# glacierbliss/iceberg_tracking_code

Hardware: AMD Instinct MI355X
Metric: frame_pairs_per_sec (higher is better)
Workload: dtype u8/int32/f32

## Files before the change

iceberg_tracking_code_amd/csrc/k_corners.hip:

```cpp
#include <algorithm>
#include <climits>
#include <cstdlib>

#include "icelk_internal.h"
#include "strip_sqrt.h"

namespace icelk {

namespace {

__device__ __forceinline__ int reflect101(int p, int n)
{
    if (n == 1) return 0;
    while (p < 0 || p >= n) p = p < 0 ? -p : 2 * n - 2 - p;
    return p;
}

__device__ __forceinline__ unsigned ordered_key(float v)
{
    const unsigned b = __float_as_uint(v);
    return (b & 0x80000000u) ? ~b : (b | 0x80000000u);
}
__device__ __forceinline__ float key_to_float(unsigned k)
{
    const unsigned b = (k & 0x80000000u) ? (k & 0x7fffffffu) : ~k;
    return __uint_as_float(b);
}

__device__ __forceinline__ unsigned pack_xy(int x, int y) { return ((unsigned)y << 16) | (unsigned)x; }

__device__ __forceinline__ float threshold_of(const unsigned* max_key, double quality)
{
    const unsigned mk = *max_key;
    const double max_val = mk ? (double)key_to_float(mk) : 0.0;
    return (float)(max_val * quality);
}

__device__ __forceinline__ float row_smooth(float a, float b, float c, float k0, float k1, int variant)
{
    if (variant & 2) return fmaf(k1, c, fmaf(k0, b, __fmul_rn(k1, a)));
    return __fadd_rn(__fadd_rn(__fmul_rn(k1, a), __fmul_rn(k0, b)), __fmul_rn(k1, c));
}

__device__ __forceinline__ void sobel_cov(float a0, float b0, float c0, float a1, float c1, float a2, float b2,
                                          float c2, float k0, float k1, float& xx, float& xy, float& yy, int variant = 0)
{
    const float dx = (variant & 1) ? fmaf(__fadd_rn(__fsub_rn(c0, a0), __fsub_rn(c2, a2)), k1, __fmul_rn(__fsub_rn(c1, a1), k0))
                                   : __fadd_rn(__fmul_rn(__fadd_rn(__fsub_rn(c0, a0), __fsub_rn(c2, a2)), k1),
                                               __fmul_rn(__fsub_rn(c1, a1), k0));
    const float t0 = row_smooth(a0, b0, c0, k0, k1, variant);
    const float t2 = row_smooth(a2, b2, c2, k0, k1, variant);
    const float dy = __fsub_rn(t2, t0);
    xx = __fmul_rn(dx, dx);
    xy = __fmul_rn(dx, dy);
    yy = __fmul_rn(dy, dy);
}

typedef float f2 __attribute__((ext_vector_type(2)));
__device__ __forceinline__ void sobel_cov2(f2 a0, f2 b0, f2 c0, f2 a1, f2 c1, f2 a2, f2 b2, f2 c2, float k0, float k1,
                                           f2& xx, f2& xy, f2& yy)
{
    const f2 dx = ((c0 - a0) + (c2 - a2)) * k1 + (c1 - a1) * k0;
    const f2 t0 = (a0 * k1 + b0 * k0) + c0 * k1;
    const f2 t2 = (a2 * k1 + b2 * k0) + c2 * k1;
    const f2 dy = t2 - t0;
    xx = dx * dx;
    xy = dx * dy;
    yy = dy * dy;
}

template <int N, int BS>
__device__ __forceinline__ void window_sums(const double (&v)[N + BS - 1], double (&out)[N])
{
    if constexpr (BS <= 3) {
#pragma unroll
        for (int i = 0; i < N; i++) {
            double s = 0;
#pragma unroll
            for (int k = 0; k < BS; k++) s += v[i + k];
            out[i] = s;
        }
    } else {
        double s = v[0];
#pragma unroll
        for (int k = 1; k < BS; k++) s += v[k];
        out[0] = s;
#pragma unroll
        for (int i = 1; i < N; i++) {
            s = (s - v[i - 1]) + v[i + BS - 1];
            out[i] = s;
        }
    }
}

__device__ __forceinline__ float min_eig_of(double s0, double s1, double s2, int variant = 0)
{
    const float a = __fmul_rn((float)s0, 0.5f), b = (float)s1, c = __fmul_rn((float)s2, 0.5f);
    const float d = __fsub_rn(a, c);
    const float r = (variant & 4) ? fmaf(b, b, __fmul_rn(d, d)) : __fadd_rn(__fmul_rn(d, d), __fmul_rn(b, b));
    return __fsub_rn(__fadd_rn(a, c), sqrtf(r));
}

__device__ __forceinline__ void publish_max(unsigned* max_key, unsigned best, int tid)
{
#pragma unroll
    for (int o = 32; o >= 1; o >>= 1) {
        const unsigned other = __shfl_xor(best, o);
        best = other > best ? other : best;
    }
    if ((tid & 63) == 0 && best > __atomic_load_n(max_key, __ATOMIC_RELAXED)) atomicMax(max_key, best);
}

struct CandSrc {
    const unsigned long long* keys;
    const int* blk_count;
    int nblk;
    int region;
};

constexpr int gcd_c(int a, int b) { return b == 0 ? a : gcd_c(b, a % b); }

template <int BS>
struct StripCfg {
    static constexpr int NT = 256;
    static constexpr int AN = BS / 2;
    static constexpr int EW = NT - (BS - 1);
    static constexpr int TW = EW - 2;
    static constexpr int R = 4;
    static constexpr int UNROLL = BS * R / gcd_c(BS, R);
    static constexpr int EH = (64 / UNROLL) * UNROLL;
    static constexpr int SH = EH - 2;
    static constexpr int NROWS = EH + BS - 1;
    static constexpr int RX = 4;
    static constexpr int NG = (EW + RX - 1) / RX;
    static constexpr int VP = NT + 2;
    static constexpr int SUB = 16, NSUB = (SH + SUB - 1) / SUB;
    static constexpr int V_BYTES = R * 3 * VP * 8;
    static constexpr int E_BYTES = 8 * NT * 4;
    static constexpr int LDS_BYTES = V_BYTES + E_BYTES;
    static_assert(EH % R == 0 && NG <= 64 && RX * NG <= NT + RX - 1, "one wave per row of a batch");
    static_assert(RX * (NG - 1) + RX + BS - 2 < VP, "row tasks stay inside a row of column sums");
    static_assert((VP * 8) % 16 == 0, "16-byte reads of the column sums");
};

struct PixelRow {
    __amdgpu_buffer_rsrc_t rsrc;
    unsigned at;
    __device__ __forceinline__ unsigned operator[](unsigned x) const { return __builtin_amdgcn_raw_buffer_load_b8(rsrc, x, at, 0); }
};
struct PixelRows {
    __amdgpu_buffer_rsrc_t rsrc;
    unsigned pitch;
    __device__ __forceinline__ PixelRow row(int y) const { return PixelRow{rsrc, (unsigned)y * pitch}; }
};

struct SobelRoll {
    float d1, d2, t1, t2;
};

__device__ __forceinline__ float smooth3(float a, float b, float c, float k0, float k1)
{
    return __fadd_rn(__fadd_rn(__fmul_rn(k1, a), __fmul_rn(k0, b)), __fmul_rn(k1, c));
}

template <int N, bool BAND>
__device__ __forceinline__ void min_eig_strip(const double (&Sm)[3][N], float (&e)[N])
{
    if constexpr (!BAND) {
#pragma unroll
        for (int k = 0; k < N; k++) e[k] = min_eig_of(Sm[0][k], Sm[1][k], Sm[2][k]);
        return;
    }
    float tr[N], r[N];
    unsigned lo = 0xffffffffu, hi = 0u;
#pragma unroll
    for (int k = 0; k < N; k++) {
        const float a = __fmul_rn((float)Sm[0][k], 0.5f), b = (float)Sm[1][k], c = __fmul_rn((float)Sm[2][k], 0.5f);
        const float d = __fsub_rn(a, c);
        r[k] = __fadd_rn(__fmul_rn(d, d), __fmul_rn(b, b));
        tr[k] = __fadd_rn(a, c);
        const unsigned rb = __float_as_uint(r[k]);
        lo = rb < lo ? rb : lo;
        hi = rb > hi ? rb : hi;
    }
    if (__builtin_expect(__builtin_amdgcn_ballot_w64(lo < SQRT_BAND_LO || hi > SQRT_BAND_HI) == 0, 1)) {
#pragma unroll
        for (int k = 0; k < N; k++) e[k] = __fsub_rn(tr[k], sqrt_in_band(r[k]));
    } else {
#pragma unroll
        for (int k = 0; k < N; k++) e[k] = __fsub_rn(tr[k], sqrtf(r[k]));
    }
}

template <int BS, bool FRESH, bool FAST>
__device__ __forceinline__ void strip_body(const uint8_t* __restrict__ img, int w, int h, int pitch, float k0, float k1,
                                           const uint8_t* __restrict__ mask, int mask_pitch, unsigned* __restrict__ max_key,
                                           unsigned long long* __restrict__ raw, int* __restrict__ blk_count,
                                           float* __restrict__ eig_out, uint8_t* smem, int* s_cnt)
{
    using C = StripCfg<BS>;
    double* Vb = reinterpret_cast<double*>(smem);
    float* Er = reinterpret_cast<float*>(smem + C::V_BYTES);
    const int tid = threadIdx.x;
    const int x0 = blockIdx.x * C::TW, y0 = blockIdx.y * C::SH;
    const int xs = x0 - 1 - C::AN, ys = y0 - 1 - C::AN;
    const int rx = reflect101(xs + tid, w);
    const unsigned xm = (unsigned)reflect101(rx - 1, w), xc = (unsigned)rx, xp = (unsigned)reflect101(rx + 1, w);
    const PixelRows px{__builtin_amdgcn_make_buffer_rsrc(const_cast<uint8_t*>(img), 0, pitch * h, 0x00020000), (unsigned)pitch};
    const int bid = blockIdx.y * gridDim.x + blockIdx.x;
    if (tid < C::NSUB) s_cnt[tid] = 0;
    if (tid < C::R * 3 * (C::VP - C::NT)) Vb[(tid / (C::VP - C::NT)) * C::VP + C::NT + tid % (C::VP - C::NT)] = 0.0;

    float ring[3][BS];
#pragma unroll
    for (int k = 0; k < BS; k++) ring[0][k] = ring[1][k] = ring[2][k] = 0.f;
    double V[3] = {0.0, 0.0, 0.0};
    SobelRoll S{};
    unsigned pa = 0, pb = 0, pc = 0;
    if (!FRESH) {
        const PixelRow r2 = px.row(ys - 1), r1 = px.row(ys), r0 = px.row(ys + 1);
        const float a2 = (float)r2[xm], b2 = (float)r2[xc], c2 = (float)r2[xp];
        const float a1 = (float)r1[xm], b1 = (float)r1[xc], c1 = (float)r1[xp];
        S.d2 = __fsub_rn(c2, a2); S.t2 = smooth3(a2, b2, c2, k0, k1);
        S.d1 = __fsub_rn(c1, a1); S.t1 = smooth3(a1, b1, c1, k0, k1);
        pa = r0[xm]; pb = r0[xc]; pc = r0[xp];
    }
    auto cov_row = [&](int r, float& xx, float& xy, float& yy) {
        float dtop, dmid, dbot, ttop, tbot;
        if (FRESH) {
            const int ry = reflect101(ys + r, h);
            const PixelRow q0 = px.row(reflect101(ry - 1, h)), q1 = px.row(ry), q2 = px.row(reflect101(ry + 1, h));
            const float a0 = (float)q0[xm], b0 = (float)q0[xc], c0 = (float)q0[xp];
            const float a1 = (float)q1[xm], c1 = (float)q1[xp];
            const float a2 = (float)q2[xm], b2 = (float)q2[xc], c2 = (float)q2[xp];
            dtop = __fsub_rn(c0, a0); dmid = __fsub_rn(c1, a1); dbot = __fsub_rn(c2, a2);
            ttop = smooth3(a0, b0, c0, k0, k1); tbot = smooth3(a2, b2, c2, k0, k1);
        } else {
            float a = (float)pa, b = (float)pb, c = (float)pc;
            asm("" : "+v"(a), "+v"(c));
            int nr = ys + r + 2;
            nr = nr < h ? nr : h - 1;
            const PixelRow q = px.row(nr);
            pa = q[xm]; pb = q[xc]; pc = q[xp];
            dtop = S.d2; dmid = S.d1; dbot = __fsub_rn(c, a);
            ttop = S.t2; tbot = smooth3(a, b, c, k0, k1);
            S.d2 = S.d1; S.d1 = dbot; S.t2 = S.t1; S.t1 = tbot;
        }
        const float dx = __fadd_rn(__fmul_rn(__fadd_rn(dtop, dbot), k1), __fmul_rn(dmid, k0));
        const float dy = __fsub_rn(tbot, ttop);
        xx = __fmul_rn(dx, dx); xy = __fmul_rn(dx, dy); yy = __fmul_rn(dy, dy);
    };

#pragma unroll
    for (int r = 0; r < BS - 1; r++) {
        float p[3];
        cov_row(r, p[0], p[1], p[2]);
#pragma unroll
        for (int q = 0; q < 3; q++) { V[q] += (double)p[q]; ring[q][r] = p[q]; }
    }

    unsigned best = 0;
    constexpr int KL = C::TW - C::RX * (C::NG - 1);
    static_assert(KL >= 0 && KL < C::RX && C::RX * C::NG - 1 >= C::TW, "the last row task holds the strip's last output column");
    int top_hi[3], top_lo[3];
#pragma unroll
    for (int k = 0; k < 3; k++) { top_hi[k] = INT_MIN; top_lo[k] = INT_MAX; }
    const int wr = __builtin_amdgcn_readfirstlane(tid >> 6), g = tid & 63;
    for (int base = 0; base < C::EH; base += C::UNROLL) {
#pragma unroll
        for (int j = 0; j < C::UNROLL; j++) {
            const int i = base + j;
            const int K = (BS - 1 + j) % BS;
            float p[3];
            cov_row(BS - 1 + i, p[0], p[1], p[2]);
#pragma unroll
            for (int q = 0; q < 3; q++) {
                V[q] = (V[q] + (double)p[q]) - (double)ring[q][K];
                ring[q][K] = p[q];
                Vb[((j % C::R) * 3 + q) * C::VP + tid] = V[q];
            }
            __builtin_amdgcn_sched_barrier(0);
            if (j % C::R != C::R - 1) continue;
            const int eb = i / C::R;
            __syncthreads();
            if (g < C::NG && wr < C::R) {
                double Sm[3][C::RX];
#pragma unroll
                for (int q = 0; q < 3; q++) {
                    double v[C::RX + BS - 1];
                    const double* src = Vb + (wr * 3 + q) * C::VP + C::RX * g;
#pragma unroll
                    for (int k = 0; k < C::RX + BS - 1; k++) v[k] = src[k];
                    window_sums<C::RX, BS>(v, Sm[q]);
                    __builtin_amdgcn_sched_barrier(0);
                }
                const int er = eb * C::R + wr;
                float e[C::RX];
                min_eig_strip<C::RX, BS != 3>(Sm, e);
                *reinterpret_cast<float4*>(Er + (er & 7) * C::NT + C::RX * g) = make_float4(e[0], e[1], e[2], e[3]);
                const int y = y0 - 1 + er;
                if constexpr (FAST) {
                    if (er >= 1 && er <= C::SH) {
#pragma unroll
                        for (int k = 0; k < C::RX; k++) {
                            const int cls = k == 0 ? 0 : (k <= KL ? 1 : 2), bits = __float_as_int(e[k]);
                            top_hi[cls] = max(top_hi[cls], bits);
                            top_lo[cls] = min(top_lo[cls], bits);
                        }
                    }
                } else if (er >= 1 && er <= C::SH && y < h) {
#pragma unroll
                    for (int k = 0; k < C::RX; k++) {
                        const int ce = C::RX * g + k, x = x0 - 1 + ce;
                        if (ce >= 1 && ce <= C::TW && x < w) {
                            if (eig_out) eig_out[(size_t)y * w + x] = e[k];
                            if (!mask || mask[(size_t)y * mask_pitch + x]) {
                                const unsigned key = ordered_key(e[k]);
                                best = key > best ? key : best;
                            }
                        }
                    }
                }
            }
            __syncthreads();
            {
                const int x = x0 - 1 + tid;
                if (tid >= 1 && tid <= C::TW && x >= 1 && x < w - 1) {
                    float m3[6], mid[6], side[6];
#pragma unroll
                    for (int k = 0; k < 6; k++) {
                        const float* row = Er + ((eb * C::R - 2 + k) & 7) * C::NT + tid;
                        const float l = row[-1], c = row[0], r = row[1];
                        mid[k] = c;
                        side[k] = fmaxf(l, r);
                        m3[k] = fmaxf(side[k], c);
                    }
#pragma unroll
                    for (int q = 0; q < 4; q++) {
                        const int c = eb * C::R - 1 + q, y = y0 - 1 + c;
                        if (c < 1 || c > C::SH || y < 1 || y >= h - 1) continue;
                        const float v = mid[q + 1];
                        if (!(v > 0.f)) continue;
                        const float m = fmaxf(fmaxf(m3[q], m3[q + 2]), side[q + 1]);
                        if (v < m) continue;
                        if (mask && !mask[(size_t)y * mask_pitch + x]) continue;
                        const int sub = (c - 1) / C::SUB;
                        const int pos = atomicAdd(&s_cnt[sub], 1);
                        raw[((size_t)bid * C::NSUB + sub) * (C::TW * C::SUB) + pos] =
                            ((unsigned long long)ordered_key(v) << 32) | pack_xy(x, y);
                    }
                }
            }
        }
    }
    if constexpr (FAST) {
        const bool counts[3] = {g >= 1 && g < C::NG, g < C::NG, g < C::NG - 1};
        int hi = INT_MIN, lo = INT_MAX;
#pragma unroll
        for (int k = 0; k < 3; k++)
            if (counts[k]) { hi = max(hi, top_hi[k]); lo = min(lo, top_lo[k]); }
        if (lo <= hi) best = ordered_key(__int_as_float(hi >= 0 ? hi : lo));
    }
    publish_max(max_key, best, tid);
    __syncthreads();
    if (tid < C::NSUB) blk_count[bid * C::NSUB + tid] = s_cnt[tid];
}

template <int BS>
__global__ __launch_bounds__(256) __attribute__((amdgpu_waves_per_eu(3, 4))) void k_eig_strip(const uint8_t* __restrict__ img, int w, int h, int pitch, float k0,
                                                    float k1, const uint8_t* __restrict__ mask, int mask_pitch,
                                                    unsigned* __restrict__ max_key,
                                                    unsigned long long* __restrict__ raw, int* __restrict__ blk_count,
                                                    float* __restrict__ eig_out)
{
    using C = StripCfg<BS>;
    extern __shared__ __attribute__((aligned(16))) uint8_t smem[];
    __shared__ int s_cnt[C::NSUB];
    const int ys = (int)blockIdx.y * C::SH - 1 - C::AN;
    const bool rolling = ys - 1 >= 0 && ys + C::NROWS <= h - 1;
    const bool inside_x = ((int)blockIdx.x + 1) * C::TW <= w;
    if (rolling && inside_x && !mask && !eig_out)
        strip_body<BS, false, true>(img, w, h, pitch, k0, k1, mask, mask_pitch, max_key, raw, blk_count, eig_out, smem, s_cnt);
    else if (rolling)
        strip_body<BS, false, false>(img, w, h, pitch, k0, k1, mask, mask_pitch, max_key, raw, blk_count, eig_out, smem, s_cnt);
    else
        strip_body<BS, true, false>(img, w, h, pitch, k0, k1, mask, mask_pitch, max_key, raw, blk_count, eig_out, smem, s_cnt);
}

__device__ __forceinline__ void block_append(bool keep, unsigned long long key, unsigned long long* out,
                                             int* out_count, int* s_cnt, int* s_base)
{
    if (threadIdx.x == 0) *s_cnt = 0;
    __syncthreads();
    const int pos = keep ? atomicAdd(s_cnt, 1) : 0;
    __syncthreads();
    if (threadIdx.x == 0 && *s_cnt) *s_base = atomicAdd(out_count, *s_cnt);
    __syncthreads();
    if (keep) out[*s_base + pos] = key;
    __syncthreads();
}

__global__ __launch_bounds__(256) void k_flatten(CandSrc src, const unsigned* __restrict__ max_key, double quality,
                                                 unsigned long long* __restrict__ cand, int* __restrict__ cand_count)
{
    __shared__ int s_cnt, s_base;
    const float thr = threshold_of(max_key, quality);
    for (int b = blockIdx.x; b < src.nblk; b += gridDim.x) {
        const int cnt = src.blk_count[b];
        for (int i0 = 0; i0 < cnt; i0 += 256) {
            const int i = i0 + threadIdx.x;
            unsigned long long key = 0;
            bool keep = false;
            if (i < cnt) {
                key = src.keys[(size_t)b * src.region + i];
                keep = key_to_float((unsigned)(key >> 32)) > thr;
            }
            block_append(keep, key, cand, cand_count, &s_cnt, &s_base);
        }
    }
}

constexpr int EIG_TW = 64;
constexpr int EIG_TH = 16;

__global__ __launch_bounds__(256) void k_min_eig(const uint8_t* __restrict__ img, int w, int h, int pitch, int bs,
                                                 float k0, float k1, float* __restrict__ eig,
                                                 const uint8_t* __restrict__ mask, int mask_pitch,
                                                 unsigned* __restrict__ max_key, int variant)
{
    extern __shared__ __attribute__((aligned(16))) uint8_t smem[];
    const int anchor = bs / 2;
    const int ew = EIG_TW + bs - 1, eh = EIG_TH + bs - 1;
    double* hs = reinterpret_cast<double*>(smem);
    float* cov = reinterpret_cast<float*>(smem + sizeof(double) * 3 * eh * EIG_TW);
    const int x0 = blockIdx.x * EIG_TW, y0 = blockIdx.y * EIG_TH;
    const int tid = threadIdx.x;
    for (int i = tid; i < ew * eh; i += 256) {
        const int ey = i / ew, ex = i - ey * ew;
        const int rx = reflect101(x0 - anchor + ex, w), ry = reflect101(y0 - anchor + ey, h);
        const int xm = reflect101(rx - 1, w), xp = reflect101(rx + 1, w);
        const int ym = reflect101(ry - 1, h), yp = reflect101(ry + 1, h);
        const uint8_t* r0 = img + (size_t)ym * pitch;
        const uint8_t* r1 = img + (size_t)ry * pitch;
        const uint8_t* r2 = img + (size_t)yp * pitch;
        float xx, xy, yy;
        sobel_cov((float)r0[xm], (float)r0[rx], (float)r0[xp], (float)r1[xm], (float)r1[xp], (float)r2[xm],
                  (float)r2[rx], (float)r2[xp], k0, k1, xx, xy, yy, variant);
        cov[i] = xx;
        cov[ew * eh + i] = xy;
        cov[2 * ew * eh + i] = yy;
    }
    __syncthreads();
    for (int i = tid; i < eh * EIG_TW; i += 256) {
        const int ey = i / EIG_TW, ox = i - ey * EIG_TW;
        const float* c = cov + ey * ew + ox;
        double s0 = 0, s1 = 0, s2 = 0;
        for (int k = 0; k < bs; k++) {
            s0 += (double)c[k];
            s1 += (double)c[ew * eh + k];
            s2 += (double)c[2 * ew * eh + k];
        }
        hs[i] = s0;
        hs[eh * EIG_TW + i] = s1;
        hs[2 * eh * EIG_TW + i] = s2;
    }
    __syncthreads();
    unsigned best = 0;
    for (int i = tid; i < EIG_TH * EIG_TW; i += 256) {
        const int oy = i / EIG_TW, ox = i - oy * EIG_TW;
        const int x = x0 + ox, y = y0 + oy;
        if (x >= w || y >= h) continue;
        const double* r = hs + oy * EIG_TW + ox;
        double s0 = 0, s1 = 0, s2 = 0;
        for (int k = 0; k < bs; k++) {
            s0 += r[k * EIG_TW];
            s1 += r[eh * EIG_TW + k * EIG_TW];
            s2 += r[2 * eh * EIG_TW + k * EIG_TW];
        }
        const float v = min_eig_of(s0, s1, s2, variant);
        eig[(size_t)y * w + x] = v;
        if (!mask || mask[(size_t)y * mask_pitch + x]) {
            const unsigned k = ordered_key(v);
            best = k > best ? k : best;
        }
    }
    publish_max(max_key, best, tid);
}

constexpr int NMS_ROWS = 8;
__global__ __launch_bounds__(256) void k_nms_collect(const float* __restrict__ eig, int w, int h,
                                                     const uint8_t* __restrict__ mask, int mask_pitch,
                                                     const unsigned* __restrict__ max_key, double quality,
                                                     unsigned long long* __restrict__ raw, int* __restrict__ blk_count)
{
    __shared__ int list_n;
    const int tid = threadIdx.x;
    if (tid == 0) list_n = 0;
    __syncthreads();
    const int bid = blockIdx.y * gridDim.x + blockIdx.x;
    unsigned long long* region = raw + (size_t)bid * (256 * NMS_ROWS);
    const float thr = threshold_of(max_key, quality);
    const int x = blockIdx.x * 256 + tid + 1;
    for (int r = 0; r < NMS_ROWS; r++) {
        const int y = blockIdx.y * NMS_ROWS + r + 1;
        if (x >= w - 1 || y >= h - 1) continue;
        const float v = eig[(size_t)y * w + x];
        if (!(v > thr) || v == 0.f) continue;
        if (mask && !mask[(size_t)y * mask_pitch + x]) continue;
        float m = 0.f;
#pragma unroll
        for (int dy = -1; dy <= 1; dy++)
#pragma unroll
            for (int dx = -1; dx <= 1; dx++) {
                float q = eig[(size_t)(y + dy) * w + (x + dx)];
                q = q > thr ? q : 0.f;
                m = q > m ? q : m;
            }
        if (v != m) continue;
        region[atomicAdd(&list_n, 1)] = ((unsigned long long)ordered_key(v) << 32) | pack_xy(x, y);
    }
    __syncthreads();
    if (tid == 0) blk_count[bid] = list_n;
}

constexpr int CT = 64;
constexpr int SCAN_CHUNK = 2048;
constexpr int CHUNK_TOT_STRIDE = 32;

__device__ __forceinline__ void chunk_add(int* __restrict__ chunk_tot, bool active, int chunk)
{
    unsigned long long pending = __ballot(active);
    while (pending) {
        const int leader = __ffsll((long long)pending) - 1;
        const int c = __shfl(chunk, leader);
        const unsigned long long same = __ballot(active && chunk == c) & pending;
        if ((int)threadIdx.x == leader) atomicAdd(&chunk_tot[c * CHUNK_TOT_STRIDE], __popcll(same));
        pending &= ~same;
    }
}

__global__ __launch_bounds__(CT) void k_cell_count(CandSrc src, const unsigned* __restrict__ max_key, double quality,
                                                   const unsigned* __restrict__ prune_key, int w, int cell, int gw,
                                                   int* __restrict__ cell_count, int* __restrict__ chunk_tot)
{
    const float thr = threshold_of(max_key, quality);
    const unsigned pk = *prune_key;
    for (int b = blockIdx.x; b < src.nblk; b += gridDim.x) {
        const int cnt = src.blk_count[b];
        for (int i0 = 0; i0 < cnt; i0 += CT) {
            const int i = i0 + threadIdx.x;
            bool keep = false;
            int c = 0;
            if (i < cnt) {
                const unsigned long long key = src.keys[(size_t)b * src.region + i];
                keep = (unsigned)(key >> 32) >= pk && key_to_float((unsigned)(key >> 32)) > thr;
                const unsigned idx = (unsigned)key;
                const int y = (int)(idx >> 16), x = (int)(idx & 0xffffu);
                c = (y / cell) * gw + (x / cell);
            }
            if (keep) atomicAdd(&cell_count[c], 1);
            chunk_add(chunk_tot, keep, c / SCAN_CHUNK);
        }
    }
}

constexpr int KEY_SHIFT = 18;
constexpr int KEY_BINS = 2048;
__device__ __forceinline__ int key_bin(unsigned key, unsigned max_key)
{
    const int b = (int)(max_key >> KEY_SHIFT) - (int)(key >> KEY_SHIFT);
    return b < 0 ? 0 : (b >= KEY_BINS ? KEY_BINS - 1 : b);
}

__global__ __launch_bounds__(CT) void k_key_hist(CandSrc src, const unsigned* __restrict__ max_key, double quality,
                                                 unsigned* __restrict__ hist)
{
    __shared__ unsigned lh[KEY_BINS];
    for (int i = threadIdx.x; i < KEY_BINS; i += CT) lh[i] = 0;
    __syncthreads();
    const float thr = threshold_of(max_key, quality);
    const unsigned mk = *max_key;
    for (int b = blockIdx.x; b < src.nblk; b += gridDim.x) {
        const int cnt = src.blk_count[b];
        for (int i = threadIdx.x; i < cnt; i += CT) {
            const unsigned k = (unsigned)(src.keys[(size_t)b * src.region + i] >> 32);
            if (key_to_float(k) > thr) atomicAdd(&lh[key_bin(k, mk)], 1u);
        }
    }
    __syncthreads();
    for (int i = threadIdx.x; i < KEY_BINS; i += CT) {
        const unsigned v = lh[i];
        if (v) atomicAdd(&hist[i], v);
    }
}

__global__ __launch_bounds__(CT) void k_key_select(const unsigned* __restrict__ hist, unsigned want,
                                                   const unsigned* __restrict__ max_key,
                                                   unsigned* __restrict__ prune_key)
{
    constexpr int PER = KEY_BINS / CT;
    const int lane = threadIdx.x;
    unsigned s = 0;
    for (int i = 0; i < PER; i++) s += hist[lane * PER + i];
    unsigned incl = s;
#pragma unroll
    for (int o = 1; o < CT; o <<= 1) {
        const unsigned v = __shfl_up(incl, o);
        if (lane >= o) incl += v;
    }
    const unsigned total = __shfl(incl, CT - 1);
    if (lane == 0 && total < want) *prune_key = 0u;
    const unsigned above = incl - s;
    if (above < want && incl >= want) {
        unsigned run = above;
        for (int i = 0; i < PER; i++) {
            run += hist[lane * PER + i];
            if (run >= want) {
                const int bin = lane * PER + i;
                const int top = (int)(*max_key >> KEY_SHIFT);
                *prune_key = (bin >= KEY_BINS - 1 || top - bin <= 0) ? 0u : (unsigned)(top - bin) << KEY_SHIFT;
                break;
            }
        }
    }
}

__global__ __launch_bounds__(CT) void k_scan(const int* __restrict__ count, const int* __restrict__ chunk_tot,
                                             int* __restrict__ start, int n)
{
    const int lane = threadIdx.x;
    const int lo = blockIdx.x * SCAN_CHUNK;
    int run = 0;
    for (int c = lane; c < (int)blockIdx.x; c += CT) run += chunk_tot[c * CHUNK_TOT_STRIDE];
#pragma unroll
    for (int o = 32; o >= 1; o >>= 1) run += __shfl_xor(run, o);
    for (int r = 0; r < SCAN_CHUNK / (4 * CT); r++) {
        const int i0 = lo + r * 4 * CT + 4 * lane;
        int c[4], s = 0;
#pragma unroll
        for (int k = 0; k < 4; k++) {
            c[k] = i0 + k < n ? count[i0 + k] : 0;
            s += c[k];
        }
        int inc = s;
#pragma unroll
        for (int o = 1; o < CT; o <<= 1) {
            const int v = __shfl_up(inc, o);
            if (lane >= o) inc += v;
        }
        int at = run + inc - s;
#pragma unroll
        for (int k = 0; k < 4; k++) {
            if (i0 + k < n) start[i0 + k] = at;
            at += c[k];
            if (i0 + k == n - 1) start[n] = at;
        }
        run += __shfl(inc, CT - 1);
    }
    if (n == 0 && blockIdx.x == 0 && lane == 0) start[0] = 0;
}

__global__ __launch_bounds__(CT) void k_cell_fill(CandSrc src, const unsigned* __restrict__ max_key, double quality,
                                                   const unsigned* __restrict__ prune_key, int w, int cell, int gw,
                                                   const int* __restrict__ cell_start, int* __restrict__ cell_fill,
                                                   unsigned long long* __restrict__ cell_cand,
                                                   uint8_t* __restrict__ state)
{
    const float thr = threshold_of(max_key, quality);
    const unsigned pk = *prune_key;
    for (int b = blockIdx.x; b < src.nblk; b += gridDim.x) {
        const int cnt = src.blk_count[b];
        for (int i = threadIdx.x; i < cnt; i += CT) {
            const unsigned long long key = src.keys[(size_t)b * src.region + i];
            if ((unsigned)(key >> 32) < pk || !(key_to_float((unsigned)(key >> 32)) > thr)) continue;
            const unsigned idx = (unsigned)key;
            const int y = (int)(idx >> 16), x = (int)(idx & 0xffffu);
            const int c = (y / cell) * gw + (x / cell);
            const int pos = cell_start[c] + atomicAdd(&cell_fill[c], 1);
            cell_cand[pos] = key;
            state[pos] = 0;
        }
    }
}

constexpr int SUP_K = 24;
constexpr int SUP_SPINS = 48;
__global__ __launch_bounds__(CT) void k_suppress(const unsigned long long* __restrict__ cell_cand,
                                                  const int* __restrict__ n_ptr, int cell, int gw, int gh,
                                                  const int* __restrict__ cell_start, uint8_t* state, double md2,
                                                  int* __restrict__ launch_counters, int r)
{
    __shared__ int blockers[SUP_K * CT];
    if (r > 0 && launch_counters[r - 1] == 0) return;
    const int n = *n_ptr;
    int* mine = blockers + threadIdx.x;
    for (int i = blockIdx.x * blockDim.x + threadIdx.x; i < n; i += gridDim.x * blockDim.x) {
        if (__atomic_load_n(&state[i], __ATOMIC_RELAXED)) continue;
        const unsigned long long key = cell_cand[i];
        const unsigned idx = (unsigned)key;
        const int y = (int)(idx >> 16), x = (int)(idx & 0xffffu);
        const int xc = x / cell, yc = y / cell;
        const int x1 = max(0, xc - 1), y1 = max(0, yc - 1), x2 = min(gw - 1, xc + 1), y2 = min(gh - 1, yc + 1);
        int cnt = 0;
        bool rejected = false, overflow = false;
        for (int yy = y1; yy <= y2 && !rejected; yy++) {
            const int b = cell_start[yy * gw + x1], e = cell_start[yy * gw + x2 + 1];
            for (int j = b; j < e; j++) {
                const unsigned long long kj = cell_cand[j];
                if (kj <= key) continue;
                const unsigned ij = (unsigned)kj;
                const int yj = (int)(ij >> 16), xj = (int)(ij & 0xffffu);
                const float dx = (float)(x - xj), dy = (float)(y - yj);
                if (!((double)(dx * dx + dy * dy) < md2)) continue;
                const uint8_t sj = __atomic_load_n(&state[j], __ATOMIC_RELAXED);
                if (sj == 1) { rejected = true; break; }
                if (sj == 0) {
                    if (cnt < SUP_K) mine[CT * cnt++] = j;
                    else overflow = true;
                }
            }
        }
        bool decided = false;
        if (rejected) { __atomic_store_n(&state[i], (uint8_t)2, __ATOMIC_RELAXED); decided = true; }
        else if (cnt == 0 && !overflow) { __atomic_store_n(&state[i], (uint8_t)1, __ATOMIC_RELAXED); decided = true; }
        for (int spin = 0; spin < SUP_SPINS && !decided && !overflow; spin++) {
            __builtin_amdgcn_s_sleep(8);
            int k = 0;
            for (int q = 0; q < cnt; q++) {
                const int j = mine[CT * q];
                const uint8_t sj = __atomic_load_n(&state[j], __ATOMIC_RELAXED);
                if (sj == 1) { rejected = true; break; }
                if (sj == 0) mine[CT * k++] = j;
            }
            cnt = k;
            if (rejected) { __atomic_store_n(&state[i], (uint8_t)2, __ATOMIC_RELAXED); decided = true; }
            else if (cnt == 0) { __atomic_store_n(&state[i], (uint8_t)1, __ATOMIC_RELAXED); decided = true; }
        }
        if (!decided) atomicAdd(&launch_counters[r], 1);
    }
}

__global__ void k_detect_reset(int* __restrict__ cell_count, int* __restrict__ cell_fill, int ncell,
                               int* __restrict__ chunk_tot, int* __restrict__ undecided, int* __restrict__ acc_count,
                               int* __restrict__ cand_count, unsigned* __restrict__ max_key,
                               unsigned* __restrict__ key_hist, unsigned* __restrict__ prune_key, int full)
{
    const int i0 = blockIdx.x * blockDim.x + threadIdx.x;
    for (int i = i0; i <= ncell; i += gridDim.x * blockDim.x) {
        cell_count[i] = 0;
        if (i < ncell) cell_fill[i] = 0;
        if (i % SCAN_CHUNK == 0) chunk_tot[(i / SCAN_CHUNK) * CHUNK_TOT_STRIDE] = 0;
    }
    if (full & 1)
        for (int i = i0; i < KEY_BINS; i += gridDim.x * blockDim.x) key_hist[i] = 0;
    if (i0 < 8) undecided[i0] = 0;
    if (i0 == 0) {
        *acc_count = 0;
        *cand_count = 0;
        *prune_key = 0;
        if (full & 2) *max_key = 0;
    }
}

__global__ __launch_bounds__(CT) void k_gather_accepted(const unsigned long long* __restrict__ cell_cand,
                                                         const int* __restrict__ n_ptr,
                                                         const uint8_t* __restrict__ state,
                                                         unsigned long long* __restrict__ acc,
                                                         int* __restrict__ acc_count)
{
    __shared__ int s_cnt, s_base;
    const int n = *n_ptr;
    for (int i0 = blockIdx.x * CT; i0 < n; i0 += gridDim.x * CT) {
        const int i = i0 + threadIdx.x;
        const bool keep = i < n && state[i] == 1;
        block_append(keep, keep ? cell_cand[i] : 0ull, acc, acc_count, &s_cnt, &s_base);
    }
}

__global__ void k_emit(const unsigned long long* __restrict__ keys, int n, int w, float* __restrict__ xy)
{
    const int i = blockIdx.x * blockDim.x + threadIdx.x;
    if (i >= n) return;
    const unsigned idx = (unsigned)keys[i];
    const int y = (int)(idx >> 16), x = (int)(idx & 0xffffu);
    xy[2 * i] = (float)x;
    xy[2 * i + 1] = (float)y;
}

__global__ __launch_bounds__(CT) void k_tail(const unsigned long long* __restrict__ keys, int n, float* __restrict__ corners,
                                             float* __restrict__ seg_xy, uint8_t* __restrict__ seg_alive,
                                             float* __restrict__ seg_tracks, int max_vert, int emit_blocks,
                                             int* __restrict__ cell_count, int* __restrict__ cell_fill, int ncell,
                                             int* __restrict__ chunk_tot, int* __restrict__ undecided,
                                             int* __restrict__ acc_count, int* __restrict__ cand_count,
                                             unsigned* __restrict__ max_key, unsigned* __restrict__ key_hist,
                                             unsigned* __restrict__ prune_key, int full)
{
    if ((int)blockIdx.x < emit_blocks) {
        const int i = blockIdx.x * CT + threadIdx.x;
        if (i >= n) return;
        const unsigned idx = (unsigned)keys[i];
        const float x = (float)(int)(idx & 0xffffu), y = (float)(int)(idx >> 16);
        corners[2 * i] = x; corners[2 * i + 1] = y;
        seg_xy[2 * i] = x; seg_xy[2 * i + 1] = y;
        seg_alive[i] = 1;
        seg_tracks[((size_t)i * max_vert) * 2] = x;
        seg_tracks[((size_t)i * max_vert) * 2 + 1] = y;
        return;
    }
    const int i0 = ((int)blockIdx.x - emit_blocks) * CT + threadIdx.x, stride = ((int)gridDim.x - emit_blocks) * CT;
    for (int i = i0; i <= ncell; i += stride) {
        cell_count[i] = 0;
        if (i < ncell) cell_fill[i] = 0;
        if (i % SCAN_CHUNK == 0) chunk_tot[(i / SCAN_CHUNK) * CHUNK_TOT_STRIDE] = 0;
    }
    if (full & 1)
        for (int i = i0; i < KEY_BINS; i += stride) key_hist[i] = 0;
    if (i0 < 8) undecided[i0] = 0;
    if (i0 == 0) {
        *acc_count = 0;
        *cand_count = 0;
        *prune_key = 0;
        if (full & 2) *max_key = 0;
    }
}

void sobel_scale(int block_size, float* k0, float* k1)
{
    double scale = (double)(1 << 2) * block_size;
    scale *= 255.0;
    scale = 1.0 / scale;
    *k1 = (float)(1.0 * scale);
    *k0 = (float)(2.0 * scale);
}

template <int BS>
void launch_strip(hipStream_t s, const Level& img, float k0, float k1, const uint8_t* mask, int mask_pitch,
                  unsigned* max_key, unsigned long long* raw, int* blk_count, float* eig_out, CandSrc* src)
{
    using C = StripCfg<BS>;
    dim3 grid((img.w + C::TW - 1) / C::TW, (img.h + C::SH - 1) / C::SH);
    hipLaunchKernelGGL((k_eig_strip<BS>), grid, dim3(C::NT), C::LDS_BYTES, s, img.ptr, img.w, img.h, img.pitch, k0, k1, mask,
                       mask_pitch, max_key, raw, blk_count, eig_out);
    src->nblk = (int)(grid.x * grid.y) * C::NSUB;
    src->region = C::TW * C::SUB;
    src->keys = raw;
    src->blk_count = blk_count;
}

template <int BS>
void strip_geometry(int w, int h, size_t* regions, size_t* keys)
{
    using C = StripCfg<BS>;
    const size_t r = (size_t)((w + C::TW - 1) / C::TW) * ((h + C::SH - 1) / C::SH) * C::NSUB;
    const size_t k = r * (size_t)(C::TW * C::SUB);
    *regions = r > *regions ? r : *regions;
    *keys = k > *keys ? k : *keys;
}
void strip_layout(int w, int h, size_t* regions, size_t* keys)
{
    *regions = *keys = 0;
    strip_geometry<3>(w, h, regions, keys); strip_geometry<5>(w, h, regions, keys);
    strip_geometry<7>(w, h, regions, keys); strip_geometry<10>(w, h, regions, keys);
}

dim3 nms_grid(int w, int h) { return dim3((w - 2 + 255) / 256, (h - 2 + NMS_ROWS - 1) / NMS_ROWS); }

}

size_t min_eig_lds_bytes(int block_size)
{
    const int ew = EIG_TW + block_size - 1, eh = EIG_TH + block_size - 1;
    return sizeof(double) * 3 * eh * EIG_TW + sizeof(float) * 3 * eh * ew;
}

bool fused_block_size(int bs) { return bs == 3 || bs == 5 || bs == 7 || bs == 10; }

size_t candidate_capacity(int w, int h)
{
    size_t strip_r, strip_k;
    strip_layout(w, h, &strip_r, &strip_k);
    const size_t generic = (size_t)((w + 255) / 256) * ((h + NMS_ROWS - 1) / NMS_ROWS) * (256 * NMS_ROWS);
    const size_t m = std::max({generic, fast_key_capacity(w, h), strip_k});
    return m + 1024;
}
size_t candidate_blocks(int w, int h)
{
    size_t strip_r, strip_k;
    strip_layout(w, h, &strip_r, &strip_k);
    const dim3 g = nms_grid(w, h);
    const size_t m = std::max({(size_t)g.x * g.y, fast_regions(w, h), strip_r});
    return m + 16;
}

void launch_min_eig(hipStream_t s, const Level& img, int block_size, float* eig, const uint8_t* mask,
                    int mask_pitch, unsigned* max_key, int variant)
{
    float k0, k1;
    sobel_scale(block_size, &k0, &k1);
    const size_t lds = min_eig_lds_bytes(block_size);
    static size_t attr_lds = 0;
    if (lds > attr_lds) {
        hipFuncSetAttribute(reinterpret_cast<const void*>(&k_min_eig), hipFuncAttributeMaxDynamicSharedMemorySize,
                            (int)lds);
        attr_lds = lds;
    }
    dim3 grid((img.w + EIG_TW - 1) / EIG_TW, (img.h + EIG_TH - 1) / EIG_TH);
    hipLaunchKernelGGL(k_min_eig, grid, dim3(256), lds, s, img.ptr, img.w, img.h, img.pitch, block_size, k0, k1, eig,
                       mask, mask_pitch, max_key, variant);
}

static CandSrc src_of(const DetectScratch& D)
{
    CandSrc c;
    c.keys = D.cb.raw;
    c.blk_count = D.cb.blk_count;
    c.nblk = D.cb.nblk;
    c.region = D.cb.region;
    return c;
}

void launch_detect_reset(hipStream_t s, DetectScratch& D, int ncell, int mode)
{
    int blocks = (ncell + CT) / CT;
    if ((mode & 1) && blocks < KEY_BINS / CT) blocks = KEY_BINS / CT;
    if (blocks > 2048) blocks = 2048;
    hipLaunchKernelGGL(k_detect_reset, dim3(blocks), dim3(CT), 0, s, D.cell_count, D.cell_fill, ncell, D.chunk_tot, D.undecided,
                       D.acc_count, D.cand_count, D.cb.max_key, D.key_hist, D.prune_key, mode);
}

void launch_candidates(hipStream_t s, DetectScratch& D, const Level& img, int block_size, const uint8_t* mask,
                       int mask_pitch, double quality, bool use_generic, float* eig_out_or_null, int variant)
{
    if (variant) use_generic = true;
    unsigned long long* raw = D.cb.raw;
    CandSrc g_src{};
    const bool two_pass = D.cb.acand != nullptr && getenv("ICELK_TWO_PASS_CORNERS") != nullptr;
    if (two_pass && !use_generic && fused_block_size(block_size) && !eig_out_or_null &&
        launch_candidates_fast(s, D, img, block_size, mask, mask_pitch, quality))
        return;
    if (!use_generic && fused_block_size(block_size)) {
        float k0, k1;
        sobel_scale(block_size, &k0, &k1);
        switch (block_size) {
            case 3: launch_strip<3>(s, img, k0, k1, mask, mask_pitch, D.cb.max_key, raw, D.cb.blk_count, eig_out_or_null, &g_src); break;
            case 5: launch_strip<5>(s, img, k0, k1, mask, mask_pitch, D.cb.max_key, raw, D.cb.blk_count, eig_out_or_null, &g_src); break;
            case 7: launch_strip<7>(s, img, k0, k1, mask, mask_pitch, D.cb.max_key, raw, D.cb.blk_count, eig_out_or_null, &g_src); break;
            default: launch_strip<10>(s, img, k0, k1, mask, mask_pitch, D.cb.max_key, raw, D.cb.blk_count, eig_out_or_null, &g_src); break;
        }
    } else {
        launch_min_eig(s, img, block_size, D.eig, mask, mask_pitch, D.cb.max_key, variant);
        g_src.keys = raw;
        g_src.blk_count = D.cb.blk_count;
        g_src.nblk = 0;
        g_src.region = 256 * NMS_ROWS;
        if (img.w >= 3 && img.h >= 3) {
            const dim3 grid = nms_grid(img.w, img.h);
            hipLaunchKernelGGL(k_nms_collect, grid, dim3(256), 0, s, D.eig, img.w, img.h, mask, mask_pitch, D.cb.max_key,
                               quality, raw, D.cb.blk_count);
            g_src.nblk = (int)(grid.x * grid.y);
        }
    }
    D.cb.nblk = g_src.nblk;
    D.cb.region = g_src.region;
}

void launch_flatten(hipStream_t s, DetectScratch& D, double quality)
{
    hipLaunchKernelGGL(k_flatten, dim3(512), dim3(256), 0, s, src_of(D), D.cb.max_key, quality, D.cand, D.cand_count);
}

constexpr int kSuppressLaunches = 3;
static void suppress_launches(hipStream_t s, DetectScratch& D, int w, int h, double min_distance)
{
    const int cell = (int)lrint(min_distance);
    const int gw = (w + cell - 1) / cell, gh = (h + cell - 1) / cell;
    const double md2 = min_distance * min_distance;
    for (int r = 0; r < kSuppressLaunches; r++)
        hipLaunchKernelGGL(k_suppress, dim3(r < 2 ? 4096 : 512), dim3(CT), 0, s, D.cell_cand, D.cell_start + gw * gh, cell, gw, gh,
                           D.cell_start, D.state, md2, D.undecided, r);
}

static void gather_launch(hipStream_t s, DetectScratch& D, int ncell)
{
    hipLaunchKernelGGL(k_gather_accepted, dim3(1024), dim3(CT), 0, s, D.cell_cand, D.cell_start + ncell, D.state, D.acc,
                       D.acc_count);
}

TailReset tail_reset_of(DetectScratch& D, int ncell)
{
    TailReset r{};
    r.cell_count = D.cell_count;
    r.cell_fill = D.cell_fill;
    r.ncell = ncell;
    r.chunk_tot = D.chunk_tot;
    r.undecided = D.undecided;
    r.acc_count = D.acc_count;
    r.cand_count = D.cand_count;
    r.key_hist = D.key_hist;
    r.prune_key = D.prune_key;
    r.scan_chunk = SCAN_CHUNK;
    r.chunk_stride = CHUNK_TOT_STRIDE;
    r.key_bins = KEY_BINS;
    return r;
}

void launch_min_distance(hipStream_t s, DetectScratch& D, int w, int h, double min_distance, double quality,
                         int prune_want, bool no_gather)
{
    const int cell = (int)lrint(min_distance);
    const int gw = (w + cell - 1) / cell, gh = (h + cell - 1) / cell;
    const int ncell = gw * gh;
    if (prune_want > 0) {
        hipLaunchKernelGGL(k_key_hist, dim3(256), dim3(CT), 0, s, src_of(D), D.cb.max_key, quality, D.key_hist);
        hipLaunchKernelGGL(k_key_select, dim3(1), dim3(CT), 0, s, D.key_hist, (unsigned)prune_want, D.cb.max_key, D.prune_key);
    }
    hipLaunchKernelGGL(k_cell_count, dim3(4096), dim3(CT), 0, s, src_of(D), D.cb.max_key, quality, D.prune_key, w, cell, gw,
                       D.cell_count, D.chunk_tot);
    hipLaunchKernelGGL(k_scan, dim3((ncell + SCAN_CHUNK - 1) / SCAN_CHUNK), dim3(CT), 0, s, D.cell_count, D.chunk_tot,
                       D.cell_start, ncell);
    hipLaunchKernelGGL(k_cell_fill, dim3(4096), dim3(CT), 0, s, src_of(D), D.cb.max_key, quality, D.prune_key, w, cell, gw,
                       D.cell_start, D.cell_fill, D.cell_cand, D.state);
    suppress_launches(s, D, w, h, min_distance);
    if (!no_gather) gather_launch(s, D, ncell);
}

void continue_min_distance(hipStream_t s, DetectScratch& D, int w, int h, double min_distance)
{
    const int cell = (int)lrint(min_distance);
    const int ncell = ((w + cell - 1) / cell) * ((h + cell - 1) / cell);
    hipMemsetAsync(D.undecided, 0, sizeof(int) * 8, s);
    hipMemsetAsync(D.acc_count, 0, sizeof(int), s);
    suppress_launches(s, D, w, h, min_distance);
    gather_launch(s, D, ncell);
}

int suppress_launch_count() { return kSuppressLaunches; }

void launch_tail_fused(hipStream_t s, const unsigned long long* keys, int n, float* corners, float* seg_xy,
                       uint8_t* seg_alive, float* seg_tracks, int max_vert, DetectScratch& D, int ncell, int mode)
{
    const int emit_blocks = (n + CT - 1) / CT;
    int blocks = (ncell + CT) / CT;
    if ((mode & 1) && blocks < KEY_BINS / CT) blocks = KEY_BINS / CT;
    if (blocks > 2048) blocks = 2048;
    hipLaunchKernelGGL(k_tail, dim3(emit_blocks + blocks), dim3(CT), 0, s, keys, n, corners, seg_xy, seg_alive, seg_tracks,
                       max_vert, emit_blocks, D.cell_count, D.cell_fill, ncell, D.chunk_tot, D.undecided, D.acc_count,
                       D.cand_count, D.cb.max_key, D.key_hist, D.prune_key, mode);
}

void launch_emit_corners(hipStream_t s, const unsigned long long* keys, int n, int w, float* xy)
{
    if (n <= 0) return;
    hipLaunchKernelGGL(k_emit, dim3((n + CT - 1) / CT), dim3(CT), 0, s, keys, n, w, xy);
}

}
```

Baseline: 8213.

## Prefetch pixel rows deeper and schedule edge strips first in eigen kernel

The rolling path now keeps a multi-slot row prefetch ring (PF rows ahead, on by default for block sizes 5 and 10) so global loads are issued earlier and overlap the Sobel and covariance work. The border (FRESH) path loads the next row's pixels one iteration ahead. Block rows are remapped so the slower edge strips are dispatched first, which is meant to reduce tail imbalance. It also adds an env-gated timestamp probe path, and the prefetch ring costs extra registers, which may affect occupancy.

```diff
diff --git a/iceberg_tracking_code_amd/csrc/k_corners.hip b/iceberg_tracking_code_amd/csrc/k_corners.hip
--- a/iceberg_tracking_code_amd/csrc/k_corners.hip
+++ b/iceberg_tracking_code_amd/csrc/k_corners.hip
@@ -1,6 +1,8 @@
 #include <algorithm>
 #include <climits>
+#include <cstdio>
 #include <cstdlib>
+#include <vector>
 
 #include "icelk_internal.h"
 #include "strip_sqrt.h"
@@ -192,22 +194,23 @@
     }
 }
 
-template <int BS, bool FRESH, bool FAST>
+template <int BS, bool FRESH, bool FAST, int PF, bool AHEAD>
 __device__ __forceinline__ void strip_body(const uint8_t* __restrict__ img, int w, int h, int pitch, float k0, float k1,
                                            const uint8_t* __restrict__ mask, int mask_pitch, unsigned* __restrict__ max_key,
                                            unsigned long long* __restrict__ raw, int* __restrict__ blk_count,
-                                           float* __restrict__ eig_out, uint8_t* smem, int* s_cnt)
+                                           float* __restrict__ eig_out, uint8_t* smem, int* s_cnt, int sy)
 {
     using C = StripCfg<BS>;
+    static_assert(PF >= 1 && C::UNROLL % PF == 0 && PF <= C::NROWS, "the ring's slots are static in a trip; its fill stays in the strip");
     double* Vb = reinterpret_cast<double*>(smem);
     float* Er = reinterpret_cast<float*>(smem + C::V_BYTES);
     const int tid = threadIdx.x;
-    const int x0 = blockIdx.x * C::TW, y0 = blockIdx.y * C::SH;
+    const int x0 = blockIdx.x * C::TW, y0 = sy * C::SH;
     const int xs = x0 - 1 - C::AN, ys = y0 - 1 - C::AN;
     const int rx = reflect101(xs + tid, w);
     const unsigned xm = (unsigned)reflect101(rx - 1, w), xc = (unsigned)rx, xp = (unsigned)reflect101(rx + 1, w);
     const PixelRows px{__builtin_amdgcn_make_buffer_rsrc(const_cast<uint8_t*>(img), 0, pitch * h, 0x00020000), (unsigned)pitch};
-    const int bid = blockIdx.y * gridDim.x + blockIdx.x;
+    const int bid = sy * gridDim.x + blockIdx.x;
     if (tid < C::NSUB) s_cnt[tid] = 0;
     if (tid < C::R * 3 * (C::VP - C::NT)) Vb[(tid / (C::VP - C::NT)) * C::VP + C::NT + tid % (C::VP - C::NT)] = 0.0;
 
@@ -216,32 +219,54 @@
     for (int k = 0; k < BS; k++) ring[0][k] = ring[1][k] = ring[2][k] = 0.f;
     double V[3] = {0.0, 0.0, 0.0};
     SobelRoll S{};
-    unsigned pa = 0, pb = 0, pc = 0;
+    unsigned pre[PF][3] = {};
+    unsigned nx[8] = {};
+    auto fresh_rows = [&](int r, unsigned (&o)[8]) {
+        const int ry = reflect101(ys + r, h);
+        const PixelRow q0 = px.row(reflect101(ry - 1, h)), q1 = px.row(ry), q2 = px.row(reflect101(ry + 1, h));
+        o[0] = q0[xm]; o[1] = q0[xc]; o[2] = q0[xp];
+        o[3] = q1[xm]; o[4] = q1[xp];
+        o[5] = q2[xm]; o[6] = q2[xc]; o[7] = q2[xp];
+    };
+    if (FRESH && AHEAD) fresh_rows(0, nx);
     if (!FRESH) {
         const PixelRow r2 = px.row(ys - 1), r1 = px.row(ys), r0 = px.row(ys + 1);
         const float a2 = (float)r2[xm], b2 = (float)r2[xc], c2 = (float)r2[xp];
         const float a1 = (float)r1[xm], b1 = (float)r1[xc], c1 = (float)r1[xp];
         S.d2 = __fsub_rn(c2, a2); S.t2 = smooth3(a2, b2, c2, k0, k1);
         S.d1 = __fsub_rn(c1, a1); S.t1 = smooth3(a1, b1, c1, k0, k1);
-        pa = r0[xm]; pb = r0[xc]; pc = r0[xp];
-    }
-    auto cov_row = [&](int r, float& xx, float& xy, float& yy) {
+        pre[0][0] = r0[xm]; pre[0][1] = r0[xc]; pre[0][2] = r0[xp];
+#pragma unroll
+        for (int k = 1; k < PF; k++) {
+            const PixelRow q = px.row(ys + 1 + k);
+            pre[k][0] = q[xm]; pre[k][1] = q[xc]; pre[k][2] = q[xp];
+        }
+    }
+    auto cov_row = [&](int r, int slot, float& xx, float& xy, float& yy) {
         float dtop, dmid, dbot, ttop, tbot;
         if (FRESH) {
-            const int ry = reflect101(ys + r, h);
-            const PixelRow q0 = px.row(reflect101(ry - 1, h)), q1 = px.row(ry), q2 = px.row(reflect101(ry + 1, h));
-            const float a0 = (float)q0[xm], b0 = (float)q0[xc], c0 = (float)q0[xp];
-            const float a1 = (float)q1[xm], c1 = (float)q1[xp];
-            const float a2 = (float)q2[xm], b2 = (float)q2[xc], c2 = (float)q2[xp];
+            unsigned u[8];
+            if (AHEAD) {
+#pragma unroll
+                for (int k = 0; k < 8; k++) u[k] = nx[k];
+                fresh_rows(r + 1, nx);
+            } else {
+                fresh_rows(r, u);
+            }
+            const float a0 = (float)u[0], b0 = (float)u[1], c0 = (float)u[2];
+            const float a1 = (float)u[3], c1 = (float)u[4];
+            const float a2 = (float)u[5], b2 = (float)u[6], c2 = (float)u[7];
             dtop = __fsub_rn(c0, a0); dmid = __fsub_rn(c1, a1); dbot = __fsub_rn(c2, a2);
             ttop = smooth3(a0, b0, c0, k0, k1); tbot = smooth3(a2, b2, c2, k0, k1);
         } else {
-            float a = (float)pa, b = (float)pb, c = (float)pc;
-            asm("" : "+v"(a), "+v"(c));
-            int nr = ys + r + 2;
+            float a = (float)pre[slot][0], b = (float)pre[slot][1], c = (float)pre[slot][2];
+            if constexpr (PF > 1) asm volatile("" : "+v"(a), "+v"(b), "+v"(c));
+            else asm("" : "+v"(a), "+v"(c));
+            int nr = ys + r + 1 + PF;
             nr = nr < h ? nr : h - 1;
             const PixelRow q = px.row(nr);
-            pa = q[xm]; pb = q[xc]; pc = q[xp];
+            pre[slot][0] = q[xm]; pre[slot][1] = q[xc]; pre[slot][2] = q[xp];
+            if constexpr (PF > 1) __builtin_amdgcn_sched_barrier(0);
             dtop = S.d2; dmid = S.d1; dbot = __fsub_rn(c, a);
             ttop = S.t2; tbot = smooth3(a, b, c, k0, k1);
             S.d2 = S.d1; S.d1 = dbot; S.t2 = S.t1; S.t1 = tbot;
@@ -254,7 +279,7 @@
 #pragma unroll
     for (int r = 0; r < BS - 1; r++) {
         float p[3];
-        cov_row(r, p[0], p[1], p[2]);
+        cov_row(r, r % PF, p[0], p[1], p[2]);
 #pragma unroll
         for (int q = 0; q < 3; q++) { V[q] += (double)p[q]; ring[q][r] = p[q]; }
     }
@@ -272,7 +297,7 @@
             const int i = base + j;
             const int K = (BS - 1 + j) % BS;
             float p[3];
-            cov_row(BS - 1 + i, p[0], p[1], p[2]);
+            cov_row(BS - 1 + i, (BS - 1 + j) % PF, p[0], p[1], p[2]);
 #pragma unroll
             for (int q = 0; q < 3; q++) {
                 V[q] = (V[q] + (double)p[q]) - (double)ring[q][K];
@@ -366,25 +391,56 @@
     if (tid < C::NSUB) blk_count[bid * C::NSUB + tid] = s_cnt[tid];
 }
 
+#ifndef ICELK_EIG_PF
+#define ICELK_EIG_PF 2
+#endif
+#ifndef ICELK_EIG_EDGE
+#define ICELK_EIG_EDGE 1
+#endif
+#ifdef ICELK_EIG_PF_ALL
 template <int BS>
+constexpr int strip_pf = ICELK_EIG_PF;
+#else
+template <int BS>
+constexpr int strip_pf = (BS == 5 || BS == 10) ? ICELK_EIG_PF : 1;
+#endif
+
+__device__ __forceinline__ int strip_row_of(int by, int ny)
+{
+    if (!ICELK_EIG_EDGE || ny < 3) return by;
+    return by == 0 ? 0 : (by <= 2 ? ny - by : by - 2);
+}
+
+template <int BS, int PF, bool STAMPS>
 __global__ __launch_bounds__(256) __attribute__((amdgpu_waves_per_eu(3, 4))) void k_eig_strip(const uint8_t* __restrict__ img, int w, int h, int pitch, float k0,
                                                     float k1, const uint8_t* __restrict__ mask, int mask_pitch,
                                                     unsigned* __restrict__ max_key,
                                                     unsigned long long* __restrict__ raw, int* __restrict__ blk_count,
-                                                    float* __restrict__ eig_out)
+                                                    float* __restrict__ eig_out, unsigned long long* __restrict__ stamps)
 {
     using C = StripCfg<BS>;
+    constexpr bool AHEAD = ICELK_EIG_EDGE != 0;
     extern __shared__ __attribute__((aligned(16))) uint8_t smem[];
     __shared__ int s_cnt[C::NSUB];
-    const int ys = (int)blockIdx.y * C::SH - 1 - C::AN;
+    const int sy = strip_row_of((int)blockIdx.y, (int)gridDim.y);
+    unsigned long long* st = nullptr;
+    if constexpr (STAMPS) {
+        st = stamps + 4 * ((size_t)sy * gridDim.x + blockIdx.x);
+        if (threadIdx.x == 0) { st[0] = __builtin_amdgcn_s_memrealtime(); st[2] = __builtin_amdgcn_s_memtime(); }
+    }
+    const int ys = sy * C::SH - 1 - C::AN;
     const bool rolling = ys - 1 >= 0 && ys + C::NROWS <= h - 1;
     const bool inside_x = ((int)blockIdx.x + 1) * C::TW <= w;
     if (rolling && inside_x && !mask && !eig_out)
-        strip_body<BS, false, true>(img, w, h, pitch, k0, k1, mask, mask_pitch, max_key, raw, blk_count, eig_out, smem, s_cnt);
+        strip_body<BS, false, true, PF, AHEAD>(img, w, h, pitch, k0, k1, mask, mask_pitch, max_key, raw, blk_count, eig_out, smem, s_cnt, sy);
     else if (rolling)
-        strip_body<BS, false, false>(img, w, h, pitch, k0, k1, mask, mask_pitch, max_key, raw, blk_count, eig_out, smem, s_cnt);
+        strip_body<BS, false, false, PF, AHEAD>(img, w, h, pitch, k0, k1, mask, mask_pitch, max_key, raw, blk_count, eig_out, smem, s_cnt, sy);
     else
-        strip_body<BS, true, false>(img, w, h, pitch, k0, k1, mask, mask_pitch, max_key, raw, blk_count, eig_out, smem, s_cnt);
+        strip_body<BS, true, false, PF, AHEAD>(img, w, h, pitch, k0, k1, mask, mask_pitch, max_key, raw, blk_count, eig_out, smem, s_cnt, sy);
+    if constexpr (STAMPS) {
+        __syncthreads();
+        if (threadIdx.x == 0) { st[1] = __builtin_amdgcn_s_memrealtime(); st[3] = __builtin_amdgcn_s_memtime(); }
+    }
 }
 
 __device__ __forceinline__ void block_append(bool keep, unsigned long long key, unsigned long long* out,
@@ -840,8 +896,22 @@
 {
     using C = StripCfg<BS>;
     dim3 grid((img.w + C::TW - 1) / C::TW, (img.h + C::SH - 1) / C::SH);
-    hipLaunchKernelGGL((k_eig_strip<BS>), grid, dim3(C::NT), C::LDS_BYTES, s, img.ptr, img.w, img.h, img.pitch, k0, k1, mask,
-                       mask_pitch, max_key, raw, blk_count, eig_out);
+    static const char* st_path = getenv("ICELK_EIG_STAMPS");
+    static unsigned long long* d_st = nullptr;
+    const size_t nst = 4 * (size_t)grid.x * grid.y;
+    constexpr size_t ST_CAP = 4 * 65536;
+    if (st_path && *st_path && !d_st && hipMalloc(reinterpret_cast<void**>(&d_st), ST_CAP * 8) != hipSuccess) d_st = nullptr;
+    if (d_st && nst <= ST_CAP) {
+        hipLaunchKernelGGL((k_eig_strip<BS, strip_pf<BS>, true>), grid, dim3(C::NT), C::LDS_BYTES, s, img.ptr, img.w, img.h, img.pitch,
+                           k0, k1, mask, mask_pitch, max_key, raw, blk_count, eig_out, d_st);
+        std::vector<unsigned long long> hst(nst);
+        hipStreamSynchronize(s);
+        hipMemcpy(hst.data(), d_st, nst * 8, hipMemcpyDeviceToHost);
+        if (FILE* f = fopen(st_path, "wb")) { fwrite(hst.data(), 8, nst, f); fclose(f); }
+    } else {
+        hipLaunchKernelGGL((k_eig_strip<BS, strip_pf<BS>, false>), grid, dim3(C::NT), C::LDS_BYTES, s, img.ptr, img.w, img.h, img.pitch,
+                           k0, k1, mask, mask_pitch, max_key, raw, blk_count, eig_out, static_cast<unsigned long long*>(nullptr));
+    }
     src->nblk = (int)(grid.x * grid.y) * C::NSUB;
     src->region = C::TW * C::SUB;
     src->keys = raw;
```

After: 8276 (median of 6 runs). About the same (+0.8%).
